# AIBluefisher/DAGSfM

Measured on AMD Instinct MI355X. Metric: verified image-pairs/sec (+ RANSAC hypotheses/sec) at 4096 feats/image, higher is better.
Workload: dtype u8 matching (int8 MFMA) + f64 verification

## Files before the change

### dagsfm_amd/capi.py

```python
import ctypes
import os

import numpy as np

_HERE = os.path.dirname(os.path.abspath(__file__))
LIB_PATH = os.environ.get("DSM_LIB_PATH") or os.path.join(_HERE, "libdagsfm_mi355x.so")
CHECK_LIB_PATH = os.environ.get("DSM_CHECK_LIB_PATH") or os.path.join(_HERE, "libdagsfm_mi355x_check.so")

GATHER_LIB_PATH = os.path.join(_HERE, "libdagsfm_gather.so")

u8p = ctypes.POINTER(ctypes.c_uint8)
u32p = ctypes.POINTER(ctypes.c_uint32)
u64p = ctypes.POINTER(ctypes.c_uint64)
f32p = ctypes.POINTER(ctypes.c_float)


class DsmError(RuntimeError):
    pass


class MatchOptions(ctypes.Structure):
    _fields_ = [("max_ratio", ctypes.c_double), ("max_distance", ctypes.c_double),
                ("cross_check", ctypes.c_int32), ("max_num_matches", ctypes.c_int32)]

# ... 238 lines not shown
    return int(lib().dsm_pair_seed(id1, id2, user_seed))


def simple_pinhole(f, cx, cy, width, height, prior=True):
    c = Camera(model_id=0, has_prior_focal_length=int(bool(prior)), width=width, height=height)
    c.params[0], c.params[1], c.params[2] = f, cx, cy
    return c


CAMERA_MODEL_NUM_PARAMS = (3, 4, 4, 5, 8, 8, 12, 5, 4, 5, 12)


def camera(model_id, params, width, height, prior=True):
    c = Camera(model_id=model_id, has_prior_focal_length=int(bool(prior)), width=width, height=height)
    for k, v in enumerate(params):
        c.params[k] = float(v)
    return c


def default_match_options(**kw):
    o = MatchOptions()
    lib().dsm_default_match_options(ctypes.byref(o))
    for k, v in kw.items():
        setattr(o, k, v)
    return o


def default_two_view_options(**kw):
    o = TwoViewOptions()
    lib().dsm_default_two_view_options(ctypes.byref(o))
    for k, v in kw.items():
        setattr(o, k, v)
    return o


def default_rotation_averaging_options(**kw):
    o = RotationAveragingOptions()
    lib().dsm_default_rotation_averaging_options(ctypes.byref(o))
    for k, v in kw.items():
        setattr(o, k, v)
    return o


def default_clustering_options(**kw):
    o = ClusteringOptions()
    lib().dsm_default_clustering_options(ctypes.byref(o))
    for k, v in kw.items():
        setattr(o, k, v)
    return o


def default_align_options(**kw):
    o = AlignOptions()
    lib().dsm_default_align_options(ctypes.byref(o))
    for k, v in kw.items():
        setattr(o, k, v)
    return o


def default_bundle_adjustment_options(**kw):
    o = BundleAdjustmentOptions()
    lib().dsm_default_bundle_adjustment_options(ctypes.byref(o))
    for k, v in kw.items():
        setattr(o, k, v)
    return o


def default_triangulation_options(**kw):
    o = TriangulationOptions()
    lib().dsm_default_triangulation_options(ctypes.byref(o))
    for k, v in kw.items():
        setattr(o, k, v)
    return o


def align_seed(i, j, direction, user_seed=0):
    return int(lib().dsm_align_seed(i, j, direction, user_seed))


PRODUCT_OPTION_KEYS = ("DSM_MATCH_CHUNK_ROWS", "DSM_VERIFY_CHUNK_PAIRS", "DSM_VERIFY_LANES", "DSM_VERIFY_INLINE_LO", "DSM_VERIFY_ITEM_MODE",
                       "DSM_LO_TAIL", "DSM_LO_TAIL_MODE", "DSM_VERIFY_GRID_DIV")
CHECK_OPTION_KEYS = ("DSM_K1_DOT4", "DSM_VERIFY_DEBUG", "DSM_SAMPLER_SERIAL", "DSM_LO_PREPARE_WAVE", "DSM_LO_JACOBI_GROUPS", "DSM_ROOTS_LDS",
                     "DSM_FINAL_WAVES", "DSM_VERIFY_LEGACY", "DSM_VERIFY_FIXED_BATCH", "DSM_VERIFY_LANE_SPLIT", "DSM_DEBUG_SAMPLER_MODE",
                     "DSM_VOCAB_ASSIGN_VALU", "DSM_VERIFY_HOST_LOOP", "DSM_SCORE_PREFILTER", "DSM_VERIFY_REPLAY_GRID", "DSM_REPLAY_LEGACY", "DSM_FLANN_GROUP", "DSM_FLANN_STATS", "DSM_ELU_LDS", "DSM_HYP_GRID", "DSM_SPEC_MARGIN")
DEBUG_OPTION_KEYS = PRODUCT_OPTION_KEYS


def check_requested():
    return os.environ.get("DSM_LIBRARY") == "check" or any(os.environ.get(k) is not None for k in CHECK_OPTION_KEYS)


class Context:

    def __init__(self, device=0, check=None):
        self._handle = ctypes.c_void_p()
        self._debug = {}
        self.check = check_requested() if check is None else bool(check)
        self._L = lib(self.check)
        rc = self._L.dsm_ctx_create(device, ctypes.byref(self._handle))
        if rc != 0:
            raise DsmError("dsm_ctx_create failed (%d): %s" % (rc, self._L.dsm_last_error(None).decode()))
        self.n_pairs = 0

    @property
    def _h(self):
        if self._handle:
            for key in PRODUCT_OPTION_KEYS + CHECK_OPTION_KEYS:
                want = os.environ.get(key)
                if self._debug.get(key) != want:
                    self.set_debug_option(key, want)
        return self._handle

    def set_memory_budget(self, nbytes):
        self._L.dsm_ctx_set_memory_budget.argtypes = [ctypes.c_void_p, ctypes.c_uint64]
        self._chk(self._L.dsm_ctx_set_memory_budget(self._handle, ctypes.c_uint64(int(nbytes))))

    def memory_footprint(self):
        r, s = ctypes.c_uint64(0), ctypes.c_uint64(0)
        self._L.dsm_ctx_memory_footprint.argtypes = [ctypes.c_void_p, ctypes.POINTER(ctypes.c_uint64), ctypes.POINTER(ctypes.c_uint64)]
        self._chk(self._L.dsm_ctx_memory_footprint(self._handle, ctypes.byref(r), ctypes.byref(s)))
        return int(r.value), int(s.value)

    def set_debug_option(self, key, value):
        L = self._L
        rc = L.dsm_set_debug_option(self._handle, key.encode(), None if value is None else str(value).encode())
        if rc != 0:
            raise DsmError("dsm_set_debug_option(%s) failed (%d)" % (key, rc))
        if value is None:
            self._debug.pop(key, None)
        else:
            self._debug[key] = str(value)

    def close(self):
        if self._handle:
            self._L.dsm_ctx_destroy(self._handle)
            self._handle = ctypes.c_void_p()

    def __del__(self):
        try:
            self.close()
        except Exception:
            pass

    def _chk(self, rc):
        if rc != 0:
            raise DsmError("dsm error %d: %s" % (rc, self._L.dsm_last_error(self._h).decode()))

    def sync(self):
        self._chk(self._L.dsm_sync(self._h))

    def append_images(self, descriptors, keypoints=None, cameras=None):
        self.set_images(descriptors, keypoints, cameras, _append=True)

    def set_images(self, descriptors, keypoints=None, cameras=None, _append=False):
        n = len(descriptors)
        descs = [np.ascontiguousarray(d, dtype=np.uint8).reshape(-1, 128) for d in descriptors]
        nf = np.array([d.shape[0] for d in descs], dtype=np.uint32)
        vp = ctypes.c_void_p
        dptr = (vp * max(n, 1))(*[d.ctypes.data for d in descs])
        kptr = None
        stride = 0
        kps = None
        if keypoints is not None:
            kps = [np.ascontiguousarray(k, dtype=np.float32) for k in keypoints]
            kps = [k.reshape(-1, k.shape[-1] if k.ndim == 2 else 2) for k in kps]
            stride = kps[0].shape[1] if n else 2
            for k, d in zip(kps, descs):
# ... 437 lines not shown
```

### dagsfm_amd/csrc/capi.hip

```cpp
#include <hip/hip_runtime.h>
#include <math.h>
#include <stdint.h>
#include <stdio.h>
#include <stdlib.h>
#include <string.h>

#include <algorithm>
#include <string>
#include <system_error>
#include <thread>
#include <vector>

#include "../../include/dagsfm_mi355x.h"
#include "ctx.h"
#include "kernels.h"
#include "verify_camera.h"

namespace {
thread_local std::string g_create_error;
}

static const uint64_t kStageSlot = 16ull << 20;
static const uint64_t kStageSmall = 1ull << 20;
static const unsigned kStageThreads = 8;
// ... 958 lines not shown
  HIPCHK(ctx, ctx->d_inl_counts.reserve(std::max<uint32_t>(n_pairs, 1) * 4));
  HIPCHK(ctx, ctx->d_inl_off.reserve(((size_t)n_pairs + 1) * 8));
  HIPCHK(ctx, ctx->d_inl_total.reserve(8));
  int dev_cus = 256;
  (void)hipDeviceGetAttribute(&dev_cus, hipDeviceAttributeMultiprocessorCount, ctx->device);
  const uint32_t n_blocks = std::min<uint32_t>(n_pairs, (uint32_t)dev_cus * 16u);
  (void)n_blocks;
  const uint64_t tm = std::max<uint64_t>(total_matches, 1);
  HIPCHK(ctx, ctx->d_pair_state.reserve(std::max<size_t>(n_pairs, 1) * 1280 * 4));
  HIPCHK(ctx, ctx->d_pts_px.reserve(tm * 32));
  HIPCHK(ctx, ctx->d_pts_norm.reserve(tm * 32));
  HIPCHK(ctx, ctx->d_reports.reserve(std::max<size_t>(n_pairs, 1) * 3 * sizeof(RansacReport)));
  HIPCHK(ctx, ctx->d_masks.reserve(tm * 3));
  VerifyParams vp;
  vp.pair_state = ctx->d_pair_state.as<uint32_t>();
  vp.pts_px = ctx->d_pts_px.as<double>();
  vp.pts_norm = ctx->d_pts_norm.as<double>();
  vp.reports = ctx->d_reports.as<RansacReport>();
  vp.masks = ctx->d_masks.as<unsigned char>();
  vp.mask_stride = tm;
  vp.pairs = d_pairs;
  vp.match_off = d_match_off;
  vp.matches = d_matches;
  vp.kp = d_kp;
  vp.img_row0 = d_img_row0;
  vp.cams = d_cams;
  vp.opt = *o;
  vp.seeds = d_seeds;
  vp.nt_table = ctx->d_nt_table.as<uint32_t>();
  vp.nt_off = ctx->d_nt_off.as<uint64_t>();
  vp.nt_off_t = ctx->d_nt_off_t.as<uint64_t>();
  vp.nt_table_t = ctx->d_nt_table_t.as<uint32_t>();
  vp.wm_redo = ctx->d_wm_redo.as<uint32_t>();
  vp.wm_total = ctx->d_wm_total.as<uint32_t>();
  vp.wm_count = ctx->d_wm_count.as<uint32_t>();
  vp.final_list = nullptr;
  vp.n_final = 0;
  vp.pose_jobs = ctx->d_pose_jobs.as<PoseJob>();
  vp.max_trials[0] = ransac_ctor_max_trials(o, o->min_inlier_ratio, kMinSamples[0]);
  vp.max_trials[1] = ransac_ctor_max_trials(o, o->min_inlier_ratio, kMinSamples[1]);
  vp.max_trials[2] = ransac_ctor_max_trials(o, o->min_inlier_ratio, kMinSamples[2]);
  vp.max_trials[3] = ransac_ctor_max_trials(o, o->watermark_min_inlier_ratio, kMinSamples[3]);
  vp.tvg = ctx->d_tvg.as<dsm_two_view_geometry>();
  vp.inlier_matches = ctx->d_inl.as<uint32_t>();
  vp.inl_counts = ctx->d_inl_counts.as<uint32_t>();
  vp.scratch = nullptr;
  vp.n_pairs = n_pairs;
  vp.n_max = n_max;
  vp.stage_filter = stage_filter;
  vp.sampler_serial = ctx->dbg("DSM_SAMPLER_SERIAL") ? 1 : 0;
  vp.reseed = reseed ? 1 : 0;
  vp.keep_generator = keep_generator ? 1 : 0;
  if (!ctx->vev0) HIPCHK(ctx, hipEventCreate(&ctx->vev0.e));
  if (!ctx->vev1) HIPCHK(ctx, hipEventCreate(&ctx->vev1.e));
  vp.pair0 = 0;
  vp.n_chunk = n_pairs;
  vp.batch = 0;
  vp.fam_state = nullptr;
  vp.samples = nullptr;
  vp.draws_end = nullptr;
  vp.nmodels = nullptr;
  vp.counts = nullptr;
  vp.sums = nullptr;
  vp.first_batch[0] = vp.first_batch[1] = vp.first_batch[2] = 0;
  vp.stats = ctx->dbg("DSM_VERIFY_DEBUG") ? 1 : 0;
  vp.lo_reg_prepare = ctx->dbg("DSM_LO_PREPARE_WAVE") ? 0 : 1;
  vp.rp_cap = std::min<uint32_t>(n_max, 256u);
  vp.spec_margin[0] = 8;
  vp.spec_margin[1] = vp.spec_margin[2] = 4;
  if (const char* e = ctx->dbg("DSM_SPEC_MARGIN")) {
    unsigned a = 8, b = 4;
    if (sscanf(e, "%u,%u", &a, &b) == 2) {
      vp.spec_margin[0] = a;
      vp.spec_margin[1] = b;
    }
  }
  vp.hyp_map = nullptr;
  vp.hyp_seg_cap = 0;
  vp.replay_legacy = ctx->dbg("DSM_REPLAY_LEGACY") ? 1 : 0;
  vp.dbg_elu_lds = ctx->dbg("DSM_ELU_LDS") ? 1 : 0;
  vp.dbg_jacobi_groups = ctx->dbg("DSM_LO_JACOBI_GROUPS") ? 1 : 0;
  vp.dbg_roots_lds = ctx->dbg("DSM_ROOTS_LDS") ? 1 : 0;
  vp.dbg_final_waves = ctx->dbg("DSM_FINAL_WAVES") ? atoi(ctx->dbg("DSM_FINAL_WAVES")) : 0;
  vp.score_prefilter = ctx->dbg("DSM_SCORE_PREFILTER") ? atoi(ctx->dbg("DSM_SCORE_PREFILTER")) : 1;
  const bool prefilter_check = ctx->dbg("DSM_SCORE_PREFILTER") && strcmp(ctx->dbg("DSM_SCORE_PREFILTER"), "check") == 0;
  if (prefilter_check) {
    vp.score_prefilter = 5;
    vp.stats = 1;
  }
  vp.models = nullptr;
  vp.e_work = nullptr;
  vp.sidx_g = nullptr;
  vp.active_count = nullptr;
  vp.lo_inl = nullptr;
  vp.worklist = nullptr;
  vp.n_work = 0;
  vp.lo_queue_g = nullptr;
  vp.lo_queue = nullptr;
  vp.lo_count = nullptr;
  vp.lo_work = vp.lo_models = vp.lo_slots = vp.lo_ework = nullptr;
  vp.tail_items = nullptr;
  vp.tail_n = nullptr;
  vp.lo_jobs = nullptr;
  vp.lo_inl_pool = nullptr;
  vp.job_list = nullptr;
#ifdef DSM_CHECK_BUILD
  const bool legacy = ctx->dbg("DSM_VERIFY_LEGACY") != nullptr;
#else
  const bool legacy = false;
#endif
  if (legacy) {
#ifdef DSM_CHECK_BUILD
    HIPCHK(ctx, ctx->d_vscratch.reserve(std::max<size_t>(1, (size_t)n_blocks * verify_scratch_bytes_per_block(n_max))));
    vp.scratch = ctx->d_vscratch.as<double>();
    HIPCHK(ctx, ctx->lanes[0].active.reserve(LANE_CTR_BYTES));
    HIPCHK(ctx, hipMemsetAsync(ctx->lanes[0].active.p, 0, LANE_CTR_BYTES, st));
    vp.active_count = ctx->lanes[0].active.as<uint32_t>() + LANE_CTR_AREA / 4;
    HIPCHK(ctx, hipEventRecord(ctx->vev0, st));
    launch_verify(vp, n_blocks, st);
    HIPCHK(ctx, hipGetLastError());
#endif
  } else {
    VerifyPlan plan;
    for (int f = 0; f < 3; ++f) {
      plan.batch[f] = vp_batch(f, vp.max_trials[f], (uint32_t)std::min<uint64_t>(o->min_num_trials, 0xffffffffull));
      vp.first_batch[f] = plan.batch[f];
    }
    auto per_pair_bytes = [&](const uint32_t* b, uint32_t* bmax_out, uint64_t* bm_out) {
      uint32_t bmax = 0;
      uint64_t bm = 0;
      for (int f = 0; f < 3; ++f) {
        bmax = std::max(bmax, b[f]);
        bm = std::max<uint64_t>(bm, (uint64_t)b[f] * vp_maxm(f));
      }
      if (bmax_out) *bmax_out = bmax;
      if (bm_out) *bm_out = bm;
      return (uint64_t)bmax * (7 * 4 + 4 + 4) + bm * (4 + 8 + 72) + (uint64_t)b[0] * 200 * 8 + (LO_WORK_DOUBLES + 90 + 90 + 200) * 8 + 12 + (uint64_t)std::max(b[0], b[1]) * 4;
    };
    uint32_t n_lanes = n_pairs >= 1024 ? 2 : 1;
    if (const char* e = ctx->dbg("DSM_VERIFY_LANES")) n_lanes = (uint32_t)std::max(1, std::min(DSM_VERIFY_MAX_LANES, atoi(e)));
    n_lanes = std::max<uint32_t>(1, std::min<uint32_t>(n_lanes, n_pairs));
    uint64_t budget = 16ull << 30;
    {
      size_t free_b = 0, total_b = 0;
      if (hipMemGetInfo(&free_b, &total_b) == hipSuccess) {
        uint64_t have = 0;
        for (VerifyLane& L : ctx->lanes)
          for (DevBuf* b : {&L.samples, &L.draws_end, &L.nmodels, &L.vcounts, &L.vsums, &L.models, &L.ework, &L.lo_work, &L.lo_models, &L.lo_slots,
                            &L.lo_ework})
            have += b->cap;
        budget = std::min<uint64_t>(96ull << 30, std::max<uint64_t>(4ull << 30, (uint64_t)((free_b + have) * 0.4)));
      }
    }
    if (ctx->memory_budget) budget = ctx->memory_budget - match_budget_share(ctx->memory_budget);
    if (!ctx->dbg("DSM_VERIFY_FIXED_BATCH")) {
      for (bool grew = true; grew;) {
        grew = false;
        for (int f = 1; f >= 0; --f) {
          const uint32_t cap = f == 0 ? 512u : 1024u;
          if (plan.batch[f] * 2 > cap) continue;
          uint32_t trial[3] = {plan.batch[0], plan.batch[1], plan.batch[2]};
          trial[f] *= 2;
          if (per_pair_bytes(trial, nullptr, nullptr) * (uint64_t)n_pairs <= budget / 4) {
            plan.batch[f] = trial[f];
            grew = true;
          }
// ... 718 lines not shown
```

### dagsfm_amd/csrc/ctx.h

```cpp
#ifndef DAGSFM_AMD_CSRC_CTX_H_
#define DAGSFM_AMD_CSRC_CTX_H_

#include <hip/hip_runtime.h>
#include <stdint.h>

#include <map>
#include <string>
#include <vector>

#include "../../include/dagsfm_mi355x.h"

struct DevBuf {
  void* p = nullptr;
  size_t cap = 0;
  DevBuf() = default;
  DevBuf(const DevBuf&) = delete;
  DevBuf& operator=(const DevBuf&) = delete;
  DevBuf(DevBuf&& o) noexcept : p(o.p), cap(o.cap) {
    o.p = nullptr;
    o.cap = 0;
  }
  DevBuf& operator=(DevBuf&& o) noexcept {
    if (this != &o) {
      release();
// ... 116 lines not shown
  std::vector<dsm_camera> cameras;
  bool have_kp = false;
  DevBuf d_desc, d_rterm, d_kp, d_img_row0, d_img_rows, d_lut;
  HostBuf h_stage;
  DevBuf d_stage;
  DevEvent stage_ev[2];

  bool matched = false;
  uint32_t n_pairs = 0;
  std::vector<uint32_t> pairs;
  DevBuf d_dpairs, d_doutoff, d_pair_dir, d_m, d_counts, d_offsets, d_matches, d_total;
  uint64_t total_matches = 0;
  double k1_ms = 0.0;
  double k1b_ms = 0.0;
  double k1t_ms = 0.0;
  double k1g_ms = 0.0;
  DevBuf d_order, d_dpairs2, d_ecnt, d_eoff, d_etotal, d_entries, d_out2, d_ms, d_out2s;
  uint32_t k1_launches = 0;
  std::vector<DevEvent> ev;

  bool verified = false;
  DevBuf d_cams, d_pairs_dev, d_seeds, d_tvg, d_inl, d_inl_counts, d_inl_off, d_inl_compact, d_vscratch, d_inl_total;
  DevBuf d_nt_table, d_nt_off, d_nt_off_t, d_pair_state, d_pts_px, d_pts_norm, d_reports, d_masks;
  DevBuf d_fam_state, d_sidx, d_lo_inl;
  DevBuf d_nt_table_t, d_wm_redo, d_wm_total, d_wm_count, d_lo_inl_pool, d_pose_jobs;
  VerifyLane lanes[DSM_VERIFY_MAX_LANES];
  uint32_t verify_lanes = 1;
  uint32_t verify_lo_iters[3] = {0, 0, 0};
  DevBuf d_g_nfeat, d_g_dpairs, d_g_doff, d_g_pdir, d_g_params, d_g_m, d_g_counts, d_g_offsets, d_g_total, d_g_matches,
      d_g_plan, d_g_inl, d_g_inl_off;
  DevBuf d_mm_matches[2], d_mm_off[2], d_mm_counts, d_mm_state, d_mm_first, d_mm_acc, d_mm_keep, d_mm_total;
  uint32_t verify_rounds[3] = {0, 0, 0};
  uint64_t total_inliers = 0;
  double verify_ms = 0.0;
  double nt_confidence = -1.0;
  std::vector<uint32_t> nt_table;
  std::vector<uint64_t> nt_off;
  std::vector<uint32_t> nt_table_t;
  std::vector<uint64_t> nt_off_t;
  bool nt_dirty = true, nt_dirty_t = true;
  DevEvent vev0, vev1;

  dsm_ctx* leaf = nullptr;

  std::map<std::string, std::string> debug_options;
  const char* dbg(const char* key) const {
    const auto it = debug_options.find(key);
    return it == debug_options.end() ? nullptr : it->second.c_str();
  }

  uint64_t memory_budget = 0;

  struct RetrievalState* retrieval = nullptr;

  std::vector<double> cluster_ritz, cluster_vectors;
  uint32_t cluster_rows = 0, cluster_cols = 0;

  template <typename F>
  void for_each_buffer(F f) {
    for (DevBuf* b : {&d_desc, &d_rterm, &d_kp, &d_img_row0, &d_img_rows, &d_lut, &d_stage, &d_counts, &d_offsets, &d_matches, &d_total, &d_etotal,
                      &d_cams, &d_pairs_dev, &d_seeds, &d_tvg, &d_inl, &d_inl_counts, &d_inl_off, &d_inl_compact, &d_inl_total, &d_nt_table,
                      &d_nt_off, &d_nt_off_t, &d_pair_state, &d_pts_px, &d_pts_norm, &d_reports, &d_masks, &d_fam_state, &d_sidx, &d_lo_inl,
                      &d_nt_table_t, &d_wm_redo, &d_wm_total, &d_wm_count, &d_lo_inl_pool, &d_pose_jobs,
                      &d_g_nfeat, &d_g_dpairs, &d_g_doff, &d_g_pdir, &d_g_params, &d_g_m, &d_g_counts, &d_g_offsets, &d_g_total, &d_g_matches,
                      &d_g_plan, &d_g_inl, &d_g_inl_off,
                      &d_mm_matches[0], &d_mm_matches[1], &d_mm_off[0], &d_mm_off[1], &d_mm_counts, &d_mm_state, &d_mm_first, &d_mm_acc,
                      &d_mm_keep, &d_mm_total})
      f(*b, false);
    for (DevBuf* b : {&d_m, &d_ms, &d_entries, &d_out2, &d_out2s, &d_dpairs, &d_dpairs2, &d_doutoff, &d_pair_dir, &d_order, &d_ecnt, &d_eoff,
                      &d_vscratch})
      f(*b, true);
    for (VerifyLane& L : lanes) L.for_each_buffer([&f](DevBuf& b) { f(b, true); });
  }
};
void dsm_retrieval_destroy(dsm_ctx* ctx);
void dsm_retrieval_invalidate(dsm_ctx* ctx);

static const char* const dsm_product_debug_keys[] = {"DSM_MATCH_CHUNK_ROWS", "DSM_VERIFY_CHUNK_PAIRS", "DSM_VERIFY_LANES", "DSM_VERIFY_INLINE_LO",
                                                     "DSM_VERIFY_ITEM_MODE", "DSM_LO_TAIL", "DSM_LO_TAIL_MODE", "DSM_VERIFY_GRID_DIV"};
#ifdef DSM_CHECK_BUILD
static const char* const dsm_check_debug_keys[] = {"DSM_K1_DOT4", "DSM_VERIFY_DEBUG", "DSM_SAMPLER_SERIAL", "DSM_LO_PREPARE_WAVE", "DSM_LO_JACOBI_GROUPS",
                                                   "DSM_ROOTS_LDS", "DSM_FINAL_WAVES", "DSM_VERIFY_LEGACY", "DSM_VERIFY_FIXED_BATCH", "DSM_VERIFY_LANE_SPLIT",
                                                   "DSM_DEBUG_SAMPLER_MODE", "DSM_VOCAB_ASSIGN_VALU", "DSM_VERIFY_HOST_LOOP", "DSM_SCORE_PREFILTER",
                                                   "DSM_VERIFY_REPLAY_GRID", "DSM_REPLAY_LEGACY", "DSM_FLANN_GROUP", "DSM_FLANN_STATS", "DSM_ELU_LDS", "DSM_HYP_GRID", "DSM_SPEC_MARGIN"};
#endif

#define HIPCHK(ctx, call)                                                              \
  do {                                                                                 \
    hipError_t e_ = (call);                                                            \
    if (e_ != hipSuccess) {                                                            \
      (ctx)->err = std::string(#call) + ": " + hipGetErrorString(e_);                  \
      return DSM_ERR_HIP;                                                              \
    }                                                                                  \
  } while (0)

#define HIPTRY(call)                                                   \
  do {                                                                 \
    hipError_t e_ = (call);                                            \
    if (e_ != hipSuccess && rc == DSM_OK) {                            \
      ctx->err = std::string(#call) + ": " + hipGetErrorString(e_);    \
      rc = DSM_ERR_HIP;                                                \
    }                                                                  \
  } while (0)

static inline int dsm_fail(dsm_ctx* ctx, int code, const char* msg) {
  if (ctx) ctx->err = msg;
  return code;
}

#endif
```

### dagsfm_amd/csrc/kernels.h

```cpp
#ifndef DAGSFM_AMD_CSRC_KERNELS_H_
#define DAGSFM_AMD_CSRC_KERNELS_H_

#include <hip/hip_runtime.h>
#include <stdint.h>

#include "../../include/dagsfm_mi355x.h"

struct K1Params {
  const int8_t* desc;
  const int32_t* rterm;
  const uint2* dpairs;
  const uint32_t* img_row0;
  const uint32_t* img_rows;
  const uint64_t* d_out_off;
  const float* lut;
  float max_ratio;
  float max_distance;
  int32_t* out;
  int32_t* out_s;
  const uint32_t* order;
  const uint2* entries;
  const uint64_t* e_off;
  const uint32_t* e_cnt;
};
// ... 47 lines not shown

struct FamState {
  RansacReport rep;
  uint32_t dyn_max;
  uint32_t active;
  uint32_t rounds;
  uint32_t nb;
  uint32_t t_pos;
  uint32_t m_pos;
  uint32_t lo_wait;
  uint32_t lo_ninl;
  uint32_t lo_nm;
  uint32_t pad;
};
#define LO_WORK_DOUBLES 176

#define TAIL_KMAX 8
struct PoseJob {
  int32_t ncmb;
  int32_t ni;
  double Rc[4 * 9];
  double tc[4 * 3];
  int32_t cnt[4];
  double med[4];
};
struct LoJob {
  uint32_t pl;
  uint32_t ninl;
  uint32_t pending;
  uint32_t nm;
};
struct TailItem {
  uint32_t t, m;
  uint32_t nlo;
  uint32_t out_n;
  double out_sum;
  double out_model[9];
};

#ifndef DSM_REPLAY_WAVES
#define DSM_REPLAY_WAVES 4
#endif

struct VerifyParams {
  const uint32_t* pairs;
  const uint64_t* match_off;
  const uint32_t* matches;
  const double* kp;
  const uint32_t* img_row0;
  const dsm_camera* cams;
  dsm_two_view_options opt;
  const uint32_t* seeds;
  const uint32_t* nt_table;
  const uint64_t* nt_off;
  const uint32_t* nt_table_t;
  const uint64_t* nt_off_t;
  uint32_t* wm_redo;
  uint32_t* wm_total;
  uint32_t* wm_count;
  const uint32_t* final_list;
  PoseJob* pose_jobs;
  uint32_t n_final;
  uint32_t max_trials[4];
  uint32_t first_batch[3];
  dsm_two_view_geometry* tvg;
  uint32_t* inlier_matches;
  uint32_t* inl_counts;
  double* scratch;
  uint32_t* pair_state;
  double* pts_px;
  double* pts_norm;
  RansacReport* reports;
  unsigned char* masks;
  uint64_t mask_stride;
  struct FamState* fam_state;
  uint32_t* samples;
  uint32_t* draws_end;
  int32_t* nmodels;
  int32_t* counts;
  double* sums;
  int lo_reg_prepare;
  int dbg_elu_lds;
  int dbg_jacobi_groups, dbg_roots_lds, dbg_final_waves;
  int score_prefilter;
  int stats;
  uint32_t spec_margin[3];
  uint32_t* hyp_map;
  uint32_t hyp_seg_cap;
  uint32_t rp_cap;
  int replay_legacy;
  double* models;
  uint32_t* sidx_g;
  uint32_t* active_count;
  uint32_t pair0, n_chunk;
  uint32_t batch;
  uint32_t n_pairs;
  uint32_t n_max;
  int32_t stage_filter;
  double* e_work;
  int32_t sampler_serial;
  int32_t reseed;
  int32_t keep_generator;
  uint32_t* lo_inl;
  TailItem* tail_items;
  uint32_t* tail_n;
  struct LoJob* lo_jobs;
  uint32_t* lo_inl_pool;
  uint32_t* job_list;
  const uint32_t* worklist;
  uint32_t n_work;
  uint32_t* lo_queue_g;
  uint32_t* lo_queue;
  uint32_t* lo_count;
  double* lo_work;
  double* lo_models;
  double* lo_slots;
  double* lo_ework;
};

size_t verify_scratch_bytes_per_block(uint32_t n_max);
size_t verify_smem_bytes(uint32_t n_max);
void launch_verify(const VerifyParams& p, uint32_t n_blocks, hipStream_t st);
void launch_vp_prep(const VerifyParams& p, uint32_t n_blocks, hipStream_t st);
void launch_vp_sample(const VerifyParams& p, int fam, uint32_t n_blocks, hipStream_t st);
void launch_vp_solve_score(const VerifyParams& p, int fam, hipStream_t st);
void launch_vp_replay(const VerifyParams& p, int fam, uint32_t n_blocks, hipStream_t st);
void launch_vp_final(const VerifyParams& p, uint32_t n_blocks, hipStream_t st);
void launch_vp_replay_lo(const VerifyParams& p, int fam, uint32_t n_blocks, int mode, hipStream_t st);
void launch_vp_items_enum(const VerifyParams& p, int fam, hipStream_t st);
void launch_vp_items_inliers(const VerifyParams& p, int fam, uint32_t n_blocks, hipStream_t st);
void launch_vp_items_outcome(const VerifyParams& p, int fam, uint32_t n_blocks, hipStream_t st);
void launch_vp_local_opt(const VerifyParams& p, int fam, uint32_t n_blocks, uint32_t n_wave_prepare, uint32_t n_small_jacobi, uint32_t n_big_prepare, hipStream_t st);
void launch_lane_counters(const void* src, uint32_t* dst_host, uint32_t copy_bytes, void* zero, size_t zero_bytes, hipStream_t st);
uint32_t vp_batch(int fam, uint32_t max_trials, uint32_t min_trials);
uint32_t vp_maxm(int fam);
void debug_read_prof(unsigned long long* out16);
void launch_debug_samples(uint32_t seed, uint32_t k, uint32_t total, uint32_t n_draws, uint32_t* out, uint32_t* idx, uint32_t* tmp7,
                          int mode, hipStream_t st);
void launch_debug_image_to_world(const dsm_camera& cam, uint32_t n, const double* xy, double* uv, hipStream_t st);
void launch_compact_inliers(const uint64_t* match_off, const uint64_t* inl_off, const uint32_t* inl_counts,
                            const uint32_t* src, uint32_t* dst, uint32_t n_pairs, hipStream_t st);

void launch_k0(const uint8_t* in_u8, int8_t* out_s8, int32_t* rterm, uint64_t n_rows, hipStream_t st);
void launch_k1(const K1Params& p, uint32_t n_directed, uint32_t max_row_blocks, hipStream_t st);
void launch_k1_dot4(const K1Params& p, uint32_t n_directed, uint32_t max_row_blocks, hipStream_t st);
void launch_k1_resolve(const K1Params& p, uint32_t n_directed, uint32_t max_row_blocks, hipStream_t st);
void launch_k2(const K2Params& p, uint32_t n_pairs, bool write, hipStream_t st);
void launch_k2_entries(const K2eParams& p, uint32_t n_pairs, bool write, hipStream_t st);
void launch_scan(const uint32_t* counts, uint64_t* offsets, uint32_t n, uint64_t* running_total, hipStream_t st);

struct MultiState {
  uint32_t ngeo;
  uint32_t done;
  uint32_t acc_inl;
  uint32_t pad;
  uint32_t trials[4], models[4];
};
struct MultiParams {
  const uint64_t* cur_off;
  const uint32_t* cur_matches;
  const uint64_t* orig_off;
  const dsm_two_view_geometry* tvg;
  const uint32_t* inl;
  const uint32_t* inl_counts;
  MultiState* state;
  dsm_two_view_geometry* first;
// ... 19 lines not shown
```

### dagsfm_amd/csrc/verify_kernels.hip

```cpp
#include <hip/hip_runtime.h>
#include <stddef.h>
#include <stdint.h>

#include "../../include/dagsfm_mi355x.h"
#include "kernels.h"
#include "verify_estimators.h"
#include "verify_camera.h"
#include "verify_fivept_coop.h"

#define BATCH 64

struct MtState {
  uint32_t mt[624];
  int mti;
  uint32_t calls;
};

struct VSmem {
  WvSvdShared svd;
  double sv[9];
  double lo_models[90];
  double cur_model[9];
  double bcast[16];
  int ibcast[8];
// ... 1304 lines not shown
            }
          if (m3_det(Ur) < 0)
            for (int i = 0; i < 9; ++i) Ur[i] *= -1;
          if (m3_det(Vt) < 0)
            for (int i = 0; i < 9; ++i) Vt[i] *= -1;
          const double W[9] = {0, 1, 0, -1, 0, 0, 0, 0, 1};
          double Wt[9], T1[9], R1[9], R2[9];
          m3_transpose(W, Wt);
          m3_mul(Ur, W, T1);
          m3_mul(T1, Vt, R1);
          m3_mul(Ur, Wt, T1);
          m3_mul(T1, Vt, R2);
          const double u2[3] = {Ur[2], Ur[5], Ur[8]};
          double t0[3];
          normalized3(u2, t0);
          for (int k = 0; k < 9; ++k) {
            Rc[0 * 9 + k] = R1[k];
            Rc[1 * 9 + k] = R2[k];
            Rc[2 * 9 + k] = R1[k];
            Rc[3 * 9 + k] = R2[k];
          }
          for (int k = 0; k < 3; ++k) {
            tc[0 * 3 + k] = t0[k];
            tc[1 * 3 + k] = t0[k];
            tc[2 * 3 + k] = -t0[k];
            tc[3 * 3 + k] = -t0[k];
          }
          ncmb = 4;
        } else {
          double K1[9], K2[9];
          calibration_matrix(cam1, K1);
          calibration_matrix(cam2, K2);
          ncmb = decompose_homography(Hm, K1, K2, Rc, tc);
        }
        if (lane == 0) {
          PoseJob* job = p.pose_jobs + pi;
          job->ncmb = ncmb;
          job->ni = ni;
          for (int k = 0; k < 36; ++k) job->Rc[k] = Rc[k];
          for (int k = 0; k < 12; ++k) job->tc[k] = tc[k];
        }
        pose_pending = true;
      }
    }
    if (!pose_pending && lane == 0) p.pose_jobs[pi].ncmb = 0;

    if (p.keep_generator && gen_loaded) {
      wv_sync();
      generator_store(&sm->gen, p.pair_state + (size_t)pi * PAIR_STATE_WORDS, lane);
    }
    if (p.stage_filter && (uint64_t)num_inliers < o.min_num_inliers) {
      config = DSM_CONFIG_UNDEFINED;
      for (int k = 0; k < 9; ++k) Em[k] = Fm[k] = Hm[k] = 0.0;
      for (int k = 0; k < 4; ++k) qvec[k] = 0.0;
      for (int k = 0; k < 3; ++k) tvec[k] = 0.0;
      tri_angle = 0;
      num_inliers = 0;
    }
    if (lane == 0) {
      out->config = config;
      out->num_inliers = num_inliers;
      out->num_matches = (uint32_t)n;
      out->reserved = 0;
      for (int k = 0; k < 9; ++k) {
        out->F[k] = Fm[k];
        out->E[k] = Em[k];
        out->H[k] = Hm[k];
      }
      for (int k = 0; k < 4; ++k) out->qvec[k] = qvec[k];
      for (int k = 0; k < 3; ++k) out->tvec[k] = tvec[k];
      out->tri_angle = tri_angle;
      p.inl_counts[pi] = num_inliers;
      for (int k = 0; k < 4; ++k) {
        out->num_trials[k] = ntr[k];
        out->num_models[k] = nmo[k];
      }
    }
  }
}

#ifndef K_FINAL_POSE_WAVES
#define K_FINAL_POSE_WAVES 3
#endif
__global__ __launch_bounds__(64, K_FINAL_POSE_WAVES) void k_final_pose(const VerifyParams p) {
  const int lane = threadIdx.x;
  const WgScratch ws = wg_scratch(p);
  double* pts3d = ws.pts3d_a;
  constexpr int kAngLds = 1024;
  __shared__ double s_ang[kAngLds];
  const uint32_t n_items = (p.final_list ? p.n_final : p.n_chunk) * 4u;
  for (uint32_t idx = blockIdx.x; idx < n_items; idx += gridDim.x) {
    const uint32_t pi = p.final_list ? p.final_list[idx >> 2] : p.pair0 + (idx >> 2);
    const int c = (int)(idx & 3u);
    PoseJob* job = p.pose_jobs + pi;
    if (c >= job->ncmb) continue;
    wv_sync();
    const uint64_t moff = p.match_off[pi];
    const double* ipts = p.pts_norm + 4 * moff;
    double R[9], t[3];
    for (int k = 0; k < 9; ++k) R[k] = job->Rc[c * 9 + k];
    for (int k = 0; k < 3; ++k) t[k] = job->tc[c * 3 + k];
    const int cnt = check_cheirality(R, t, ipts, job->ni, pts3d, lane);
    double med = 0.0;
    if (cnt > 0) {
      double c2[3];
      for (int i = 0; i < 3; ++i) c2[i] = -(R[0 * 3 + i] * t[0] + R[1 * 3 + i] * t[1] + R[2 * 3 + i] * t[2]);
      const double c1[3] = {-(1.0 * 0.0 + 0.0 * 0.0 + 0.0 * 0.0), -(0.0 * 0.0 + 1.0 * 0.0 + 0.0 * 0.0), -(0.0 * 0.0 + 0.0 * 0.0 + 1.0 * 0.0)};
      double baseline2 = 0;
      for (int i = 0; i < 3; ++i) baseline2 += (c1[i] - c2[i]) * (c1[i] - c2[i]);
      auto median_of_angles = [&](double* ang) {
        for (int j = lane; j < cnt; j += 64) {
          const double* X = pts3d + 3 * (size_t)j;
          double r1 = 0, r2 = 0;
          for (int k = 0; k < 3; ++k) {
            r1 += (X[k] - c1[k]) * (X[k] - c1[k]);
            r2 += (X[k] - c2[k]) * (X[k] - c2[k]);
          }
          const double ray1 = sqrt(r1), ray2 = sqrt(r2);
          const double angle = fabs(acos((ray1 * ray1 + ray2 * ray2 - baseline2) / (2 * ray1 * ray2)));
          ang[j] = isnan(angle) ? 0.0 : (angle < M_PI - angle ? angle : M_PI - angle);
        }
        wv_sync();
        const int mid = cnt / 2;
        double lo_v = 0.0, hi_v = 0.0;
        for (int b0 = 0; b0 < cnt; b0 += 64) {
          const int j = b0 + lane;
          bool is_mid = false, is_lo = false;
          double a = 0.0;
          if (j < cnt) {
            a = ang[j];
            int rank = 0;
            for (int k = 0; k < cnt; ++k) {
              const double b = ang[k];
              rank += (b < a) || (b == a && k < j);
            }
            is_mid = rank == mid;
            is_lo = rank == mid - 1;
          }
          const unsigned long long bm = __ballot(is_mid), bl = __ballot(is_lo);
          if (bm) hi_v = __shfl(a, __ffsll((long long)bm) - 1);
          if (bl) lo_v = __shfl(a, __ffsll((long long)bl) - 1);
        }
        return (cnt % 2 == 0) ? (hi_v + lo_v) / 2.0 : hi_v;
      };
      med = cnt <= kAngLds ? median_of_angles(s_ang) : median_of_angles(ws.resid);
    }
    if (lane == 0) {
      job->cnt[c] = cnt;
      job->med[c] = med;
    }
  }
}

__global__ __launch_bounds__(64) void k_final_finish(const VerifyParams p) {
  const uint32_t n_items = p.final_list ? p.n_final : p.n_chunk;
  const uint32_t idx = blockIdx.x * 64u + threadIdx.x;
  if (idx >= n_items) return;
  const uint32_t pi = p.final_list ? p.final_list[idx] : p.pair0 + idx;
  const PoseJob* job = p.pose_jobs + pi;
  if (job->ncmb <= 0) return;
  dsm_two_view_geometry* out = p.tvg + pi;
  double Rbest[9], tvec[3] = {0, 0, 0};
  for (int k = 0; k < 9; ++k) Rbest[k] = 0.0;
  int nbest = 0, cbest = -1;
  for (int c = 0; c < job->ncmb; ++c) {
    if (job->cnt[c] >= nbest) {
      for (int k = 0; k < 9; ++k) Rbest[k] = job->Rc[c * 9 + k];
      for (int k = 0; k < 3; ++k) tvec[k] = job->tc[c * 3 + k];
      nbest = job->cnt[c];
      cbest = c;
    }
  }
  double qvec[4];
  rotation_to_quaternion(Rbest, qvec);
  double tri_angle = (nbest == 0 || cbest < 0) ? 0.0 : job->med[cbest];
  int config = out->config;
  if (config == DSM_CONFIG_PLANAR_OR_PANORAMIC) {
    const double tn = sqrt(tvec[0] * tvec[0] + tvec[1] * tvec[1] + tvec[2] * tvec[2]);
    if (tn == 0) {
      config = DSM_CONFIG_PANORAMIC;
      tri_angle = 0;
    } else {
      config = DSM_CONFIG_PLANAR;
    }
  }
  out->config = config;
  for (int k = 0; k < 4; ++k) out->qvec[k] = qvec[k];
  for (int k = 0; k < 3; ++k) out->tvec[k] = tvec[k];
  out->tri_angle = tri_angle;
}

size_t verify_scratch_bytes_per_block(uint32_t n_max) { return verify_scratch_doubles(n_max) * sizeof(double); }
size_t verify_smem_bytes(uint32_t n_max) { return ((sizeof(VSmem) + 15) / 16) * 16 + (size_t)(n_max > 0 ? n_max : 1) * 4; }

static void launch_final_pose_finish(const VerifyParams& p, uint32_t n_blocks, hipStream_t st);
#ifdef DSM_CHECK_BUILD
void launch_verify(const VerifyParams& p, uint32_t n_blocks, hipStream_t st) {
  if (p.n_pairs == 0 || n_blocks == 0) return;
  const size_t smem = verify_smem_bytes(p.n_max);
  hipLaunchKernelGGL(k_verify_prep, dim3(n_blocks), dim3(64), 0, st, p);
  hipLaunchKernelGGL(k_ransac<FAM_E>, dim3(n_blocks), dim3(64), smem, st, p);
  hipLaunchKernelGGL(k_ransac<FAM_F>, dim3(n_blocks), dim3(64), smem, st, p);
  hipLaunchKernelGGL(k_ransac<FAM_H>, dim3(n_blocks), dim3(64), smem, st, p);
  hipLaunchKernelGGL(k_verify_final<2>, dim3(n_blocks), dim3(64), smem, st, p);
  launch_final_pose_finish(p, n_blocks, st);
}
#endif

uint32_t vp_batch(int fam, uint32_t max_trials, uint32_t min_trials) {
  uint32_t b;
  if (fam == FAM_E) b = 64;
  else if (fam == FAM_F) b = 128;
  else b = ((max_trials + 63u) / 64u) * 64u;
  const uint32_t cap = fam == FAM_E ? 512u : (fam == FAM_F ? 1024u : 2048u);
  const uint32_t want = ((min_trials < max_trials ? min_trials : max_trials) + 63u) / 64u * 64u;
  if (want > b) b = want;
  return b < 64u ? 64u : (b > cap ? cap : b);
}
uint32_t vp_maxm(int fam) { return fam == FAM_E ? 10u : (fam == FAM_F ? 3u : 1u); }

#define SAMPLER_PREFIX (((sizeof(MtState) + sizeof(WvSampler) + 15) / 16) * 16)

template <int FAM>
__global__ __launch_bounds__(64) void k_sample(const VerifyParams p) {
  extern __shared__ __attribute__((aligned(16))) unsigned char smem_raw[];
  MtState* gen = reinterpret_cast<MtState*>(smem_raw);
  WvSampler* ws = reinterpret_cast<WvSampler*>(smem_raw + sizeof(MtState));
  uint32_t* sidx = reinterpret_cast<uint32_t*>(smem_raw + SAMPLER_PREFIX);
  typedef Fam<FAM> F;
  const int lane = threadIdx.x;
  SegGrab wgrab;
  const uint32_t grain = work_grain(p.n_chunk);
  uint32_t pl_static = blockIdx.x;
  for (;;) {
    wv_sync();
// ... 3036 lines not shown
      hipLaunchKernelGGL(k_solve_e_lu, grid, dim3(64), ELU_SMEM, st, p);
    else
      hipLaunchKernelGGL(k_solve_e_lu_reg, grid, dim3(64), 0, st, p);
#ifdef DSM_CHECK_BUILD
    if (p.dbg_roots_lds != 0) {
      if (p.hyp_map)
        hipLaunchKernelGGL(k_roots_e_lds<true>, grid_hyp, dim3(64), 100 * 64 * sizeof(double), st, p);
      else
        hipLaunchKernelGGL(k_roots_e_lds<false>, grid, dim3(64), 100 * 64 * sizeof(double), st, p);
    } else
#endif
    if (p.hyp_map)
      hipLaunchKernelGGL(k_roots_e<true>, grid_hyp, dim3(64), 0, st, p);
    else
      hipLaunchKernelGGL(k_roots_e<false>, grid, dim3(64), 0, st, p);
    const size_t smem2e = smem + (size_t)p.batch * 10 * 2;
    const uint32_t nb_needed_e = p.n_chunk < 256u * 32u ? p.n_chunk : 256u * 32u;
    if ((p.score_prefilter & 1) && !(p.score_prefilter & 2) && p.batch * 10 <= 65535 && smem2e <= 64 * 1024) {
#ifdef DSM_CHECK_BUILD
      if (p.score_prefilter & 32)
        hipLaunchKernelGGL(k_prescore_compact<FAM_E>, dim3(p.n_chunk, (p.batch * 10 + 63) / 64), dim3(64), smem, st, p);
      else
#endif
        hipLaunchKernelGGL(k_prescore_compact2<FAM_E>, dim3(p.n_chunk, (p.batch * 10 + 63) / 64), dim3(64), smem_c2, st, p);
      hipLaunchKernelGGL(k_score_needed<FAM_E>, dim3(nb_needed_e), dim3(64), smem2e, st, p);
#ifdef DSM_CHECK_BUILD
    } else if (p.score_prefilter & 4) {
      hipLaunchKernelGGL(k_models_score_e<true>, grid, dim3(64), smem, st, p);
#endif
    } else {
      hipLaunchKernelGGL(k_models_score_e<false>, grid, dim3(64), smem, st, p);
    }
  }
  const uint32_t nb_needed = p.n_chunk < 256u * 32u ? p.n_chunk : 256u * 32u;
  if (fam == FAM_F) {
    if (p.hyp_map)
      hipLaunchKernelGGL((k_solve<FAM_F, true>), grid_hyp, dim3(64), 0, st, p);
    else
      hipLaunchKernelGGL((k_solve<FAM_F, false>), grid, dim3(64), 0, st, p);
    const size_t smem2 = smem + (size_t)p.batch * 3 * 2;
    if (p.score_prefilter && p.batch * 3 <= 65535 && smem2 <= 64 * 1024) {
      if (p.score_prefilter & 2)
        hipLaunchKernelGGL(k_prescore<FAM_F>, dim3(p.n_chunk, (p.batch * 3 + 63) / 64), dim3(64), smem, st, p);
#ifdef DSM_CHECK_BUILD
      else if (p.score_prefilter & 32)
        hipLaunchKernelGGL(k_prescore_compact<FAM_F>, dim3(p.n_chunk, (p.batch * 3 + 63) / 64), dim3(64), smem, st, p);
#endif
      else
        hipLaunchKernelGGL(k_prescore_compact2<FAM_F>, dim3(p.n_chunk, (p.batch * 3 + 63) / 64), dim3(64), smem_c2, st, p);
      hipLaunchKernelGGL(k_score_needed<FAM_F>, dim3(nb_needed), dim3(64), smem2, st, p);
    } else {
      hipLaunchKernelGGL(k_score<FAM_F>, dim3(p.n_chunk, (p.batch * 3 + 63) / 64), dim3(64), smem, st, p);
    }
  }
  if (fam == FAM_H) {
    hipLaunchKernelGGL(k_solve<FAM_H>, grid, dim3(64), 0, st, p);
    const size_t smem2 = smem + (size_t)p.batch * 2;
    if (p.score_prefilter && p.batch <= 65535 && smem2 <= 64 * 1024) {
      const size_t smem_h2 = (size_t)(p.n_max < VP_LDS_PTS ? (p.n_max > 0 ? p.n_max : 1) : VP_LDS_PTS) * 16 + 32 + (size_t)PRESCORE_LIST_CAP * 64 * 2;
#ifdef DSM_CHECK_BUILD
      if (p.score_prefilter & 8)
        hipLaunchKernelGGL(k_prescore_h_mfma, grid, dim3(64), smem, st, p);
      else if (p.score_prefilter & 16)
        hipLaunchKernelGGL(k_prescore<FAM_H>, grid, dim3(64), smem, st, p);
      else
#endif
        hipLaunchKernelGGL(k_prescore_h2, grid, dim3(64), smem_h2, st, p);
      hipLaunchKernelGGL(k_score_needed<FAM_H>, dim3(nb_needed), dim3(64), smem2, st, p);
    } else {
      hipLaunchKernelGGL(k_score<FAM_H>, grid, dim3(64), smem, st, p);
    }
  }
}
void launch_vp_replay(const VerifyParams& p, int fam, uint32_t n_blocks, hipStream_t st) {
  if (!p.n_chunk || !n_blocks) return;
  const size_t smem = ((offsetof(VSmem, gen) + 15) / 16) * 16;
  if (fam == FAM_E) hipLaunchKernelGGL(k_replay<FAM_E>, dim3(n_blocks), dim3(64), smem, st, p);
  if (fam == FAM_F) hipLaunchKernelGGL(k_replay<FAM_F>, dim3(n_blocks), dim3(64), smem, st, p);
  if (fam == FAM_H) hipLaunchKernelGGL(k_replay<FAM_H>, dim3(n_blocks), dim3(64), smem, st, p);
}
static void launch_final_pose_finish(const VerifyParams& p, uint32_t n_blocks, hipStream_t st) {
  const uint32_t n = p.final_list ? p.n_final : p.n_chunk;
  if (!n) return;
  const uint32_t items = n * 4u;
  hipLaunchKernelGGL(k_final_pose, dim3(items < n_blocks ? items : n_blocks), dim3(64), 0, st, p);
  hipLaunchKernelGGL(k_final_finish, dim3((n + 63) / 64), dim3(64), 0, st, p);
}
void launch_vp_final(const VerifyParams& p, uint32_t n_blocks, hipStream_t st) {
  if (!p.n_pairs || !n_blocks) return;
#ifdef DSM_CHECK_BUILD
  if (p.dbg_final_waves == 1)
    hipLaunchKernelGGL(k_verify_final<1>, dim3(n_blocks), dim3(64), verify_smem_bytes(p.n_max), st, p);
  else
#endif
    hipLaunchKernelGGL(k_verify_final<2>, dim3(n_blocks), dim3(64), verify_smem_bytes(p.n_max), st, p);
  launch_final_pose_finish(p, n_blocks, st);
}

void debug_read_prof(unsigned long long* out16) {
#ifdef DSM_PROFILE_SECTIONS
  (void)hipMemcpyFromSymbol(out16, HIP_SYMBOL(g_dsm_prof), 16 * sizeof(unsigned long long));
  unsigned long long zero[16] = {0};
  (void)hipMemcpyToSymbol(HIP_SYMBOL(g_dsm_prof), zero, sizeof(zero));
#else
  for (int i = 0; i < 16; ++i) out16[i] = 0;
#endif
}

__global__ __launch_bounds__(64) void k_compact_inliers(const uint64_t* match_off, const uint64_t* inl_off,
                                                        const uint32_t* inl_counts, const uint32_t* src, uint32_t* dst,
                                                        uint32_t n_pairs) {
  for (uint32_t pi = blockIdx.x; pi < n_pairs; pi += gridDim.x) {
    const uint2* s = reinterpret_cast<const uint2*>(src) + match_off[pi];
    uint2* d = reinterpret_cast<uint2*>(dst) + inl_off[pi];
    for (uint32_t i = threadIdx.x; i < inl_counts[pi]; i += 64) d[i] = s[i];
  }
}
void launch_compact_inliers(const uint64_t* match_off, const uint64_t* inl_off, const uint32_t* inl_counts,
                            const uint32_t* src, uint32_t* dst, uint32_t n_pairs, hipStream_t st) {
  if (!n_pairs) return;
  const uint32_t blocks = n_pairs < 8192 ? n_pairs : 8192;
  hipLaunchKernelGGL(k_compact_inliers, dim3(blocks), dim3(64), 0, st, match_off, inl_off, inl_counts, src, dst, n_pairs);
}

__global__ __launch_bounds__(64) void k_multi_accumulate(const MultiParams p) {
  const int lane = threadIdx.x;
  for (uint32_t pi = blockIdx.x; pi < p.n_pairs; pi += gridDim.x) {
    MultiState* ms = p.state + pi;
    const uint64_t off = p.cur_off[pi];
    const int n = (int)(p.cur_off[pi + 1] - off);
    __syncthreads();
    if (ms->done) {
      if (lane == 0) p.next_count[pi] = 0;
      continue;
    }
    const dsm_two_view_geometry* t = p.tvg + pi;
    const int config = t->config;
    if (lane < 4) {
      ms->trials[lane] += t->num_trials[lane];
      ms->models[lane] += t->num_models[lane];
    }
    if (config == DSM_CONFIG_DEGENERATE) {
      if (lane == 0) {
        ms->done = 1;
        p.next_count[pi] = 0;
      }
      continue;
    }
    const uint32_t ninl = p.inl_counts[pi];
    const uint2* inl = reinterpret_cast<const uint2*>(p.inl) + off;
    const bool accept = !(p.ignore_watermark && config == DSM_CONFIG_WATERMARK);
    const uint32_t acc0 = ms->acc_inl, ngeo0 = ms->ngeo;
    __syncthreads();
    if (accept) {
      uint2* acc = reinterpret_cast<uint2*>(p.acc) + p.orig_off[pi] + acc0;
      for (uint32_t i = lane; i < ninl; i += 64) acc[i] = inl[i];
      if (ngeo0 == 0) {
        const uint32_t* src = reinterpret_cast<const uint32_t*>(t);
        uint32_t* dst = reinterpret_cast<uint32_t*>(p.first + pi);
        for (uint32_t i = lane; i < sizeof(dsm_two_view_geometry) / 4; i += 64) dst[i] = src[i];
      }
      if (lane == 0) {
        ms->acc_inl = acc0 + ninl;
        ms->ngeo = ngeo0 + 1;
      }
    }
    const uint2* m = reinterpret_cast<const uint2*>(p.cur_matches) + off;
    bool asc = true;
// ... 161 lines not shown
```

Measured before the change: 264,600.

## Probe cheirality per candidate pose and skip settled candidates early

Restructures final pose selection so one workgroup handles a pair and all its candidate (R,t) decompositions, instead of one workgroup per candidate. A 16-point probe per candidate picks a likely leader. The leader is evaluated first, and other candidates stop counting cheirality points once they can no longer beat the best bound. The median triangulation angle is computed only for a candidate that becomes the new best. This cuts triangulation and O(n^2) median work, but serialises candidates within a pair and reduces grid parallelism. The old full path stays as a check-build option.

```diff
diff --git a/dagsfm_amd/capi.py b/dagsfm_amd/capi.py
--- a/dagsfm_amd/capi.py
+++ b/dagsfm_amd/capi.py
@@ -344,7 +344,8 @@
                        "DSM_LO_TAIL", "DSM_LO_TAIL_MODE", "DSM_VERIFY_GRID_DIV")
 CHECK_OPTION_KEYS = ("DSM_K1_DOT4", "DSM_VERIFY_DEBUG", "DSM_SAMPLER_SERIAL", "DSM_LO_PREPARE_WAVE", "DSM_LO_JACOBI_GROUPS", "DSM_ROOTS_LDS",
                      "DSM_FINAL_WAVES", "DSM_VERIFY_LEGACY", "DSM_VERIFY_FIXED_BATCH", "DSM_VERIFY_LANE_SPLIT", "DSM_DEBUG_SAMPLER_MODE",
-                     "DSM_VOCAB_ASSIGN_VALU", "DSM_VERIFY_HOST_LOOP", "DSM_SCORE_PREFILTER", "DSM_VERIFY_REPLAY_GRID", "DSM_REPLAY_LEGACY", "DSM_FLANN_GROUP", "DSM_FLANN_STATS", "DSM_ELU_LDS", "DSM_HYP_GRID", "DSM_SPEC_MARGIN")
+                     "DSM_VOCAB_ASSIGN_VALU", "DSM_VERIFY_HOST_LOOP", "DSM_SCORE_PREFILTER", "DSM_VERIFY_REPLAY_GRID", "DSM_REPLAY_LEGACY", "DSM_FLANN_GROUP", "DSM_FLANN_STATS", "DSM_ELU_LDS", "DSM_HYP_GRID", "DSM_SPEC_MARGIN",
+                     "DSM_POSE_FULL")
 DEBUG_OPTION_KEYS = PRODUCT_OPTION_KEYS
 
 
diff --git a/dagsfm_amd/csrc/capi.hip b/dagsfm_amd/csrc/capi.hip
--- a/dagsfm_amd/csrc/capi.hip
+++ b/dagsfm_amd/csrc/capi.hip
@@ -1064,6 +1064,7 @@
   vp.dbg_jacobi_groups = ctx->dbg("DSM_LO_JACOBI_GROUPS") ? 1 : 0;
   vp.dbg_roots_lds = ctx->dbg("DSM_ROOTS_LDS") ? 1 : 0;
   vp.dbg_final_waves = ctx->dbg("DSM_FINAL_WAVES") ? atoi(ctx->dbg("DSM_FINAL_WAVES")) : 0;
+  vp.dbg_pose_full = ctx->dbg("DSM_POSE_FULL") ? 1 : 0;
   vp.score_prefilter = ctx->dbg("DSM_SCORE_PREFILTER") ? atoi(ctx->dbg("DSM_SCORE_PREFILTER")) : 1;
   const bool prefilter_check = ctx->dbg("DSM_SCORE_PREFILTER") && strcmp(ctx->dbg("DSM_SCORE_PREFILTER"), "check") == 0;
   if (prefilter_check) {
diff --git a/dagsfm_amd/csrc/ctx.h b/dagsfm_amd/csrc/ctx.h
--- a/dagsfm_amd/csrc/ctx.h
+++ b/dagsfm_amd/csrc/ctx.h
@@ -222,7 +222,8 @@
 static const char* const dsm_check_debug_keys[] = {"DSM_K1_DOT4", "DSM_VERIFY_DEBUG", "DSM_SAMPLER_SERIAL", "DSM_LO_PREPARE_WAVE", "DSM_LO_JACOBI_GROUPS",
                                                    "DSM_ROOTS_LDS", "DSM_FINAL_WAVES", "DSM_VERIFY_LEGACY", "DSM_VERIFY_FIXED_BATCH", "DSM_VERIFY_LANE_SPLIT",
                                                    "DSM_DEBUG_SAMPLER_MODE", "DSM_VOCAB_ASSIGN_VALU", "DSM_VERIFY_HOST_LOOP", "DSM_SCORE_PREFILTER",
-                                                   "DSM_VERIFY_REPLAY_GRID", "DSM_REPLAY_LEGACY", "DSM_FLANN_GROUP", "DSM_FLANN_STATS", "DSM_ELU_LDS", "DSM_HYP_GRID", "DSM_SPEC_MARGIN"};
+                                                   "DSM_VERIFY_REPLAY_GRID", "DSM_REPLAY_LEGACY", "DSM_FLANN_GROUP", "DSM_FLANN_STATS", "DSM_ELU_LDS", "DSM_HYP_GRID", "DSM_SPEC_MARGIN",
+                                                   "DSM_POSE_FULL"};
 #endif
 
 #define HIPCHK(ctx, call)                                                              \
diff --git a/dagsfm_amd/csrc/kernels.h b/dagsfm_amd/csrc/kernels.h
--- a/dagsfm_amd/csrc/kernels.h
+++ b/dagsfm_amd/csrc/kernels.h
@@ -153,6 +153,7 @@
   int lo_reg_prepare;
   int dbg_elu_lds;
   int dbg_jacobi_groups, dbg_roots_lds, dbg_final_waves;
+  int dbg_pose_full;
   int score_prefilter;
   int stats;
   uint32_t spec_margin[3];
diff --git a/dagsfm_amd/csrc/verify_kernels.hip b/dagsfm_amd/csrc/verify_kernels.hip
--- a/dagsfm_amd/csrc/verify_kernels.hip
+++ b/dagsfm_amd/csrc/verify_kernels.hip
@@ -1410,7 +1410,150 @@
 #ifndef K_FINAL_POSE_WAVES
 #define K_FINAL_POSE_WAVES 3
 #endif
+DSM_DEV double median_triangulation_angle(const double* R, const double* t, const double* pts3d, int cnt, double* ang, int lane) {
+  double c2[3];
+  for (int i = 0; i < 3; ++i) c2[i] = -(R[0 * 3 + i] * t[0] + R[1 * 3 + i] * t[1] + R[2 * 3 + i] * t[2]);
+  const double c1[3] = {-(1.0 * 0.0 + 0.0 * 0.0 + 0.0 * 0.0), -(0.0 * 0.0 + 1.0 * 0.0 + 0.0 * 0.0), -(0.0 * 0.0 + 0.0 * 0.0 + 1.0 * 0.0)};
+  double baseline2 = 0;
+  for (int i = 0; i < 3; ++i) baseline2 += (c1[i] - c2[i]) * (c1[i] - c2[i]);
+  for (int j = lane; j < cnt; j += 64) {
+    const double* X = pts3d + 3 * (size_t)j;
+    double r1 = 0, r2 = 0;
+    for (int k = 0; k < 3; ++k) {
+      r1 += (X[k] - c1[k]) * (X[k] - c1[k]);
+      r2 += (X[k] - c2[k]) * (X[k] - c2[k]);
+    }
+    const double ray1 = sqrt(r1), ray2 = sqrt(r2);
+    const double angle = fabs(acos((ray1 * ray1 + ray2 * ray2 - baseline2) / (2 * ray1 * ray2)));
+    ang[j] = isnan(angle) ? 0.0 : (angle < M_PI - angle ? angle : M_PI - angle);
+  }
+  wv_sync();
+  const int mid = cnt / 2;
+  double lo_v = 0.0, hi_v = 0.0;
+  for (int b0 = 0; b0 < cnt; b0 += 64) {
+    const int j = b0 + lane;
+    bool is_mid = false, is_lo = false;
+    double a = 0.0;
+    if (j < cnt) {
+      a = ang[j];
+      int rank = 0;
+      for (int k = 0; k < cnt; ++k) {
+        const double b = ang[k];
+        rank += (b < a) || (b == a && k < j);
+      }
+      is_mid = rank == mid;
+      is_lo = rank == mid - 1;
+    }
+    const unsigned long long bm = __ballot(is_mid), bl = __ballot(is_lo);
+    if (bm) hi_v = __shfl(a, __ffsll((long long)bm) - 1);
+    if (bl) lo_v = __shfl(a, __ffsll((long long)bl) - 1);
+  }
+  return (cnt % 2 == 0) ? (hi_v + lo_v) / 2.0 : hi_v;
+}
+
+DSM_DEV bool cheirality_point(const PoseJob* job, int c, const double* p, double* X) {
+  const double kMinDepth = DBL_EPSILON;
+  double R[9], t[3];
+  for (int k = 0; k < 9; ++k) R[k] = job->Rc[c * 9 + k];
+  for (int k = 0; k < 3; ++k) t[k] = job->tc[c * 3 + k];
+  double rt[3];
+  for (int i = 0; i < 3; ++i) rt[i] = R[0 * 3 + i] * t[0] + R[1 * 3 + i] * t[1] + R[2 * 3 + i] * t[2];
+  const double max_depth = 1000.0f * sqrt(rt[0] * rt[0] + rt[1] * rt[1] + rt[2] * rt[2]);
+  const double n1 = sqrt(0.0 * 0.0 + 0.0 * 0.0 + 1.0 * 1.0);
+  const double n2 = sqrt(R[2] * R[2] + R[5] * R[5] + R[8] * R[8]);
+  triangulate_point(R, t, p[0], p[1], p[2], p[3], X);
+  const double d1 = (0.0 * X[0] + 0.0 * X[1] + 1.0 * X[2] + 0.0 * 1.0) * n1;
+  if (d1 > kMinDepth && d1 < max_depth) {
+    const double d2 = (R[6] * X[0] + R[7] * X[1] + R[8] * X[2] + t[2] * 1.0) * n2;
+    if (d2 > kMinDepth && d2 < max_depth) return true;
+  }
+  return false;
+}
+
 __global__ __launch_bounds__(64, K_FINAL_POSE_WAVES) void k_final_pose(const VerifyParams p) {
+  const int lane = threadIdx.x;
+  const WgScratch ws = wg_scratch(p);
+  double* pts3d = ws.pts3d_a;
+  constexpr int kAngLds = 1024;
+  __shared__ double s_ang[kAngLds];
+  constexpr int kProbe = 16;
+  const int gc = lane / kProbe, gk = lane % kProbe;
+  const uint32_t n_items = p.final_list ? p.n_final : p.n_chunk;
+  for (uint32_t idx = blockIdx.x; idx < n_items; idx += gridDim.x) {
+    const uint32_t pi = p.final_list ? p.final_list[idx] : p.pair0 + idx;
+    PoseJob* job = p.pose_jobs + pi;
+    const int ncmb = job->ncmb;
+    if (ncmb <= 0) continue;
+    wv_sync();
+    const int ni = job->ni;
+    const double* ipts = p.pts_norm + 4 * p.match_off[pi];
+    const int np = ni < kProbe ? ni : kProbe;
+    double PX[3] = {0, 0, 0};
+    const bool pok = (gc < ncmb && gk < np) ? cheirality_point(job, gc, ipts + 4 * (size_t)gk, PX) : false;
+    const unsigned long long pbal = __ballot(pok);
+    int lb[4];
+    for (int c = 0; c < 4; ++c) lb[c] = __popcll((pbal >> (kProbe * c)) & 0xffffull);
+    int lead = 0;
+    for (int c = 1; c < ncmb; ++c)
+      if (lb[c] >= lb[lead]) lead = c;
+    int best_c = -1, best_cnt = -1;
+    for (int o = 0; o < ncmb; ++o) {
+      const int c = o == 0 ? lead : (o - 1 < lead ? o - 1 : o);
+      int bound = 0, cnt = 0;
+      for (int k = 0; k < ncmb; ++k) {
+        if (k == c) cnt = lb[k];
+        else bound = lb[k] > bound ? lb[k] : bound;
+      }
+      if (gc == c && pok) {
+        double* dst = pts3d + 3 * (size_t)__popcll((pbal >> (kProbe * c)) & ((1ull << gk) - 1ull));
+        dst[0] = PX[0];
+        dst[1] = PX[1];
+        dst[2] = PX[2];
+      }
+      bool settled = false;
+      for (int base = np; base < ni; base += 64) {
+        if (cnt + (ni - base) < bound) {
+          settled = true;
+          break;
+        }
+        const int i = base + lane;
+        double X[3] = {0, 0, 0};
+        const bool ok = i < ni ? cheirality_point(job, c, ipts + 4 * (size_t)i, X) : false;
+        const unsigned long long bal = __ballot(ok);
+        if (ok) {
+          double* dst = pts3d + (size_t)(cnt + __popcll(bal & ((1ull << lane) - 1ull))) * 3;
+          dst[0] = X[0];
+          dst[1] = X[1];
+          dst[2] = X[2];
+        }
+        cnt += __popcll(bal);
+      }
+      wv_sync();
+      for (int k = 0; k < 4; ++k)
+        if (k == c) lb[k] = cnt;
+      double med = 0.0;
+      if (!settled && (cnt > best_cnt || (cnt == best_cnt && c > best_c))) {
+        best_cnt = cnt;
+        best_c = c;
+        if (cnt > 0) {
+          double R[9], t[3];
+          for (int k = 0; k < 9; ++k) R[k] = job->Rc[c * 9 + k];
+          for (int k = 0; k < 3; ++k) t[k] = job->tc[c * 3 + k];
+          med = cnt <= kAngLds ? median_triangulation_angle(R, t, pts3d, cnt, s_ang, lane)
+                               : median_triangulation_angle(R, t, pts3d, cnt, ws.resid, lane);
+        }
+      }
+      wv_sync();
+      if (lane == 0) {
+        job->cnt[c] = settled ? -1 : cnt;
+        job->med[c] = med;
+      }
+    }
+  }
+}
+
+#ifdef DSM_CHECK_BUILD
+__global__ __launch_bounds__(64, K_FINAL_POSE_WAVES) void k_final_pose_full(const VerifyParams p) {
   const int lane = threadIdx.x;
   const WgScratch ws = wg_scratch(p);
   double* pts3d = ws.pts3d_a;
@@ -1430,55 +1573,16 @@
     for (int k = 0; k < 3; ++k) t[k] = job->tc[c * 3 + k];
     const int cnt = check_cheirality(R, t, ipts, job->ni, pts3d, lane);
     double med = 0.0;
-    if (cnt > 0) {
-      double c2[3];
-      for (int i = 0; i < 3; ++i) c2[i] = -(R[0 * 3 + i] * t[0] + R[1 * 3 + i] * t[1] + R[2 * 3 + i] * t[2]);
-      const double c1[3] = {-(1.0 * 0.0 + 0.0 * 0.0 + 0.0 * 0.0), -(0.0 * 0.0 + 1.0 * 0.0 + 0.0 * 0.0), -(0.0 * 0.0 + 0.0 * 0.0 + 1.0 * 0.0)};
-      double baseline2 = 0;
-      for (int i = 0; i < 3; ++i) baseline2 += (c1[i] - c2[i]) * (c1[i] - c2[i]);
-      auto median_of_angles = [&](double* ang) {
-        for (int j = lane; j < cnt; j += 64) {
-          const double* X = pts3d + 3 * (size_t)j;
-          double r1 = 0, r2 = 0;
-          for (int k = 0; k < 3; ++k) {
-            r1 += (X[k] - c1[k]) * (X[k] - c1[k]);
-            r2 += (X[k] - c2[k]) * (X[k] - c2[k]);
-          }
-          const double ray1 = sqrt(r1), ray2 = sqrt(r2);
-          const double angle = fabs(acos((ray1 * ray1 + ray2 * ray2 - baseline2) / (2 * ray1 * ray2)));
-          ang[j] = isnan(angle) ? 0.0 : (angle < M_PI - angle ? angle : M_PI - angle);
-        }
-        wv_sync();
-        const int mid = cnt / 2;
-        double lo_v = 0.0, hi_v = 0.0;
-        for (int b0 = 0; b0 < cnt; b0 += 64) {
-          const int j = b0 + lane;
-          bool is_mid = false, is_lo = false;
-          double a = 0.0;
-          if (j < cnt) {
-            a = ang[j];
-            int rank = 0;
-            for (int k = 0; k < cnt; ++k) {
-              const double b = ang[k];
-              rank += (b < a) || (b == a && k < j);
-            }
-            is_mid = rank == mid;
-            is_lo = rank == mid - 1;
-          }
-          const unsigned long long bm = __ballot(is_mid), bl = __ballot(is_lo);
-          if (bm) hi_v = __shfl(a, __ffsll((long long)bm) - 1);
-          if (bl) lo_v = __shfl(a, __ffsll((long long)bl) - 1);
-        }
-        return (cnt % 2 == 0) ? (hi_v + lo_v) / 2.0 : hi_v;
-      };
-      med = cnt <= kAngLds ? median_of_angles(s_ang) : median_of_angles(ws.resid);
-    }
+    if (cnt > 0)
+      med = cnt <= kAngLds ? median_triangulation_angle(R, t, pts3d, cnt, s_ang, lane)
+                           : median_triangulation_angle(R, t, pts3d, cnt, ws.resid, lane);
     if (lane == 0) {
       job->cnt[c] = cnt;
       job->med[c] = med;
     }
   }
 }
+#endif
 
 __global__ __launch_bounds__(64) void k_final_finish(const VerifyParams p) {
   const uint32_t n_items = p.final_list ? p.n_final : p.n_chunk;
@@ -4681,8 +4785,13 @@
 static void launch_final_pose_finish(const VerifyParams& p, uint32_t n_blocks, hipStream_t st) {
   const uint32_t n = p.final_list ? p.n_final : p.n_chunk;
   if (!n) return;
-  const uint32_t items = n * 4u;
-  hipLaunchKernelGGL(k_final_pose, dim3(items < n_blocks ? items : n_blocks), dim3(64), 0, st, p);
+#ifdef DSM_CHECK_BUILD
+  if (p.dbg_pose_full) {
+    const uint32_t items = n * 4u;
+    hipLaunchKernelGGL(k_final_pose_full, dim3(items < n_blocks ? items : n_blocks), dim3(64), 0, st, p);
+  } else
+#endif
+    hipLaunchKernelGGL(k_final_pose, dim3(n < n_blocks ? n : n_blocks), dim3(64), 0, st, p);
   hipLaunchKernelGGL(k_final_finish, dim3((n + 63) / 64), dim3(64), 0, st, p);
 }
 void launch_vp_final(const VerifyParams& p, uint32_t n_blocks, hipStream_t st) {
```

After: 274,100 (median of 6 runs). +3.6%, better.
